# NeSC-IV/sage-icp

Measured on AMD Instinct MI355X. Metric: ICP frames/sec (120k-pt scan vs 1M-pt map), higher is better.
Workload: dtype f64

## Files before the change

sage-icp_amd/csrc/icp_body.h:

```cpp
#pragma once

namespace sageicp {

#ifndef SAGE_LOOP_FLAT_MINW
#define SAGE_LOOP_FLAT_MINW 8
#endif
#ifndef SAGE_SCAN_AHEAD
#define SAGE_SCAN_AHEAD 1
#endif
#ifndef SAGE_ROW_SHIFT_LAYER
#define SAGE_ROW_SHIFT_LAYER 1
#endif
#ifndef SAGE_ROW_SHIFT_MAXW
#define SAGE_ROW_SHIFT_MAXW 4
#endif

struct PairCompact {
    uint4 a, b;
    unsigned ka, oa;
    bool ha, hb;
};
struct PairFull {
    Point4 a, b;
    unsigned ka;
// ... 12 lines not shown

__device__ __forceinline__ unsigned icp_wave_of_stripe(const IcpParams &P, int wv, unsigned &stripe_id) {
    constexpr unsigned kStripe = SAGE_ICP_STRIPE;
    const unsigned xcd = blockIdx.x & 7u, jb = blockIdx.x >> 3;
    unsigned stripe = (jb / kStripe) * 8u + xcd;
    if (P.stripe_order) {
        const unsigned nstripes = gridDim.x / kStripe;
        switch (stripe * 4u / nstripes) {
            case 0: __builtin_amdgcn_s_setprio(3); break;
            case 1: __builtin_amdgcn_s_setprio(2); break;
            case 2: __builtin_amdgcn_s_setprio(1); break;
            default: break;
        }
        stripe = P.stripe_order[stripe];
    }
    stripe_id = stripe;
    const unsigned wg = stripe * kStripe + (jb % kStripe);
    return wg * static_cast<unsigned>(kIcpWavesPerBlock) + static_cast<unsigned>(wv);
}

template <bool GIVEN>
__device__ __forceinline__ void axis_gaps(double v, int k, double vs, double sc, double fs, double (&g)[3]) {
    const double below_hi = static_cast<double>(k <= 0 ? k - 1 : k) * vs;
    const double above_lo = static_cast<double>(k >= 0 ? k + 1 : k) * vs;
    const double slack = (GIVEN ? fs : 1e-9 * vs) + 1e-13 * fabs(v);
    const double lo = fmax((v - below_hi) - slack, 0.0);
    const double hi = fmax((above_lo - v) - slack, 0.0);
    g[0] = (lo * lo) * sc;
    g[1] = 0.0;
    g[2] = (hi * hi) * sc;
}

__device__ __forceinline__ float round_up_f32(double x) {
    return __uint_as_float(__float_as_uint(static_cast<float>(x)) + 1u);
}

template <int LW>
__device__ __forceinline__ bool reduce_argmin(double best, unsigned bkey, bool valid, const uint32_t *lrow, unsigned &mkey, unsigned &woff) {
    constexpr int W = 1 << LW, SH = 5;
    const double m = seg_min_f64<W>(best);
    const unsigned mine = (best == m) ? bkey : 0xFFFFFFFFu;
    mkey = seg_min_u32<W>(mine);
    const bool found = valid && mkey != 0xFFFFFFFFu;
    woff = (lrow[found ? mkey >> 8 : 0u] >> 8) * (kUnitPoints * 32u) + ((mkey & 255u) << SH);
    return found;
}

struct LoopStaged {
    unsigned qslot;
    double fx, fy, fz, fl;
    unsigned prev_key, prev_off;
    unsigned kx, ky, kz, occ;
    int pli;
};

template <int LW, bool FUSED, bool FILT, bool PERSIST = false, bool FLATQ = false, int HALF = 0>
__device__ __forceinline__ void icp_body(const IcpParams &P, uint32_t *smem, LoopGroup *G = nullptr, const double *pose = nullptr,
                                         LoopStaged *S = nullptr) {
    static_assert(!PERSIST || FUSED, "the persistent loop always accumulates");
    static_assert(PERSIST ? (HALF == 1 || HALF == 2) : HALF == 0, "k_loop runs the pass in two halves, k_icp in one");
    constexpr int W = 1 << LW;
    constexpr int QW = 64 >> LW;
    constexpr int SH = 5;
    PROBE_NN_BEGIN(np);
    PROBE_DELAY_BEGIN(t0);
    int lane;
    if constexpr (PERSIST) {
        unsigned l;
        asm volatile("v_mbcnt_lo_u32_b32 %0, -1, 0\n\tv_mbcnt_hi_u32_b32 %0, -1, %0" : "=v"(l));
        lane = static_cast<int>(l);
    } else {
        lane = static_cast<int>(threadIdx.x & 63u);
    }
    const int wv = __builtin_amdgcn_readfirstlane(static_cast<int>(threadIdx.x >> 6));
    if (FUSED && !PERSIST) {
        if (threadIdx.x == 0) {
            smem[kWgArrive] = 0u;
            smem[kWgGo] = 0u;
        }
        if (threadIdx.x < 2u * kWgAccWords) smem[kWgAcc + threadIdx.x] = 0u;
        if (threadIdx.x < 12u && !(P.chain && P.chain_iter > 0))
            reinterpret_cast<double *>(smem + kWgPose)[threadIdx.x] = threadIdx.x < 9u ? P.st->R[threadIdx.x] : P.st->T[4u + threadIdx.x - 9u];
        __syncthreads();
    }
    uint32_t *wl;
    if constexpr (PERSIST) wl = G->rows;
    else wl = smem + kWgHeaderWords + static_cast<unsigned>(wv) * icp_wave_words(LW);

    unsigned wave_id, stripe_id = 0u;
    if constexpr (PERSIST) wave_id = G->slot;
    else wave_id = icp_wave_of_stripe(P, wv, stripe_id);

    const int qw = lane >> LW;
    const unsigned ci = static_cast<unsigned>(lane) & (W - 1u);
    unsigned q, qslot = 0u, bslot = 0u;
    if constexpr (PERSIST) {
        if constexpr (HALF == 1) {
            bslot = G->perm[G->unit * (QW / 4) + static_cast<unsigned>(qw >> 2)];
            qslot = bslot * 4u + (static_cast<unsigned>(qw) & 3u);
        } else {
            qslot = S->qslot;
        }
        q = G->q_first + qslot;
    } else {
        q = wave_id * QW + static_cast<unsigned>(qw);
    }
    const bool valid = q < static_cast<unsigned>(P.n);
    const unsigned qc = valid ? q : 0u;
    uint32_t *lrow = wl + (PERSIST ? qslot : static_cast<unsigned>(qw)) * kRowLdsStride;
    const uint32_t *grow = P.rows + static_cast<size_t>(qc) * kRowWords;

    const __amdgpu_buffer_rsrc_t pts = __builtin_amdgcn_make_buffer_rsrc(
        const_cast<Point4 *>(P.pts), 0, static_cast<int>(P.pts_bytes), 0x00020000);

    const __amdgpu_buffer_rsrc_t cands = __builtin_amdgcn_make_buffer_rsrc(
        const_cast<uint4 *>(P.cand), 0, static_cast<int>(P.cand_bytes), 0x00020000);
    constexpr int SHC = FILT ? 4 : 5;

    constexpr int NP = (7 + W - 1) / W;
    uint4 rk;
    uint2 prev = make_uint2(0xFFFFFFFFu, 0u);
    Point4 f;
    uint4 pc0 = make_uint4(0u, 0u, 0u, 0u), pc1 = pc0, pc2 = pc0, pc3 = pc0, pc4 = pc0, pc5 = pc0, pc6 = pc0;
    uint32_t *lst = nullptr;
    if constexpr (PERSIST) {
        lst = G->state + qslot * kLoopStateWords;
        if constexpr (HALF == 1) {
            const uint4 fa = *reinterpret_cast<const uint4 *>(lst), fb = *reinterpret_cast<const uint4 *>(lst + 4);
            const uint4 pk = *reinterpret_cast<const uint4 *>(lst + kStPrev);
            const uint2 ko = *reinterpret_cast<const uint2 *>(lst + kStPrev + 4);
            S->qslot = qslot;
            S->fx = __hiloint2double(static_cast<int>(fa.y), static_cast<int>(fa.x));
            S->fy = __hiloint2double(static_cast<int>(fa.w), static_cast<int>(fa.z));
            S->fz = __hiloint2double(static_cast<int>(fb.y), static_cast<int>(fb.x));
            S->fl = __hiloint2double(static_cast<int>(fb.w), static_cast<int>(fb.z));
            S->prev_key = pk.x; S->prev_off = pk.y;
            S->kx = pk.z; S->ky = pk.w; S->kz = ko.x; S->occ = ko.y;
            S->pli = static_cast<int>(S->fl);
            return;
        }
        f.x = S->fx; f.y = S->fy; f.z = S->fz; f.l = S->fl;
        prev = make_uint2(S->prev_key, S->prev_off);
        rk = make_uint4(S->kx, S->ky, S->kz, S->occ);
    } else {
        rk = *reinterpret_cast<const uint4 *>(grow + kRowKey);
        if (FUSED) prev = P.nn_prev[qc];
        f = P.frame[qc];
        auto row_piece = [&](int k) {
            const unsigned p = min(ci + static_cast<unsigned>(W * k), 6u);
            return *reinterpret_cast<const uint4 *>(grow + 4u * p);
        };
        pc0 = row_piece(0); pc1 = pc0; pc2 = pc0; pc3 = pc0; pc4 = pc0; pc5 = pc0; pc6 = pc0;
        if (NP > 1) pc1 = row_piece(1);
        if (NP > 2) pc2 = row_piece(2);
        if (NP > 3) pc3 = row_piece(3);
        if (NP > 4) pc4 = row_piece(4);
        if (NP > 5) pc5 = row_piece(5);
        if (NP > 6) pc6 = row_piece(6);
    }
    PROBE_DELAY_WAIT(P, t0);
    if constexpr (FUSED && !PERSIST) {
        if (P.chain && P.chain_iter > 0) {
            if (wv == 0) chain_wait_pose(P, smem, lane);
            __syncthreads();
            if (smem[kWgGo]) return;
        }
    }
    PROBE_LOOP_POSE_USE(PERSIST, G);
    const Query s = [&]() {
        if constexpr (PERSIST) {
            return make_query<(W >= 4)>(f, pose, pose + 9, 1, P.voxel_size, P.inv_voxel_size, static_cast<unsigned>(lane));
        } else if constexpr (FUSED) {
            const double *lpose = reinterpret_cast<const double *>(smem + kWgPose);
            return make_query<(W >= 4)>(f, lpose, lpose + 9, P.apply_pose, P.voxel_size, P.inv_voxel_size, threadIdx.x);
        } else {
            return make_query<(W >= 4)>(f, P.st->R, P.st->T + 4, P.apply_pose, P.voxel_size, P.inv_voxel_size, threadIdx.x);
        }
    }();
    const bool stale = valid && (static_cast<uint32_t>(s.kx) != rk.x || static_cast<uint32_t>(s.ky) != rk.y ||
                                 static_cast<uint32_t>(s.kz) != rk.z);
    unsigned occ = rk.w;
    NN_T(np, 0);
    LP_T(PERSIST, G, 0);
    if constexpr (!PERSIST) {
        auto stage = [&](int k, const uint4 &v) {
            const unsigned p = ci + static_cast<unsigned>(W * k);
            if (p < 7u) *reinterpret_cast<uint4 *>(lrow + 4u * p) = v;
        };
        stage(0, pc0);
        if (NP > 1) stage(1, pc1);
        if (NP > 2) stage(2, pc2);
        if (NP > 3) stage(3, pc3);
        if (NP > 4) stage(4, pc4);
// ... 103 lines not shown
                        for (int j = j0; j < j0 + NB && j < NV; ++j) {
                            const int v = static_cast<int>(ci) + W * j;
                            if (reuse[j]) tally(v, ow[j]);
                            else finish(v, sl[j], e[j]);
                        }
                    }
                }
                if (nearv && prev.x != 0xFFFFFFFFu) {
                    const int vo = static_cast<int>(prev.x >> 8);
                    const int a = vo / 9 - dx, b = (vo / 3) % 3 - dy, c = vo % 3 - dz;
                    const bool in = static_cast<unsigned>(a) <= 2u && static_cast<unsigned>(b) <= 2u &&
                                    static_cast<unsigned>(c) <= 2u;
                    prev.x = in ? (static_cast<unsigned>(a * 9 + b * 3 + c) << 8) | (prev.x & 255u) : 0xFFFFFFFFu;
                } else {
                    prev.x = 0xFFFFFFFFu;
                }
            } else {
                prev.x = 0xFFFFFFFFu;
#pragma unroll 1
                for (int k0 = 0; k0 < NV; k0 += 3) {
                    const int v0 = static_cast<int>(ci) + W * k0;
                    const int v1 = k0 + 1 < NV ? v0 + W : 27, v2 = k0 + 2 < NV ? v0 + 2 * W : 27;
                    uint32_t s0, s1, s2;
                    int4 e0, e1, e2;
                    start(v0, s0, e0);
                    start(v1, s1, e1);
                    start(v2, s2, e2);
                    finish(v0, s0, e0);
                    finish(v1, s1, e1);
                    finish(v2, s2, e2);
                }
            }
            o = seg_or_u32<W>(o);
            cq = seg_add_u32<W>(cq);
            occ = o;
            if (ci == 0u) {
                lrow[kRowCq] = cq;
                if constexpr (!PERSIST) {
                    uint4 t;
                    t.x = static_cast<uint32_t>(s.kx); t.y = static_cast<uint32_t>(s.ky);
                    t.z = static_cast<uint32_t>(s.kz); t.w = o;
                    *reinterpret_cast<uint4 *>(P.rows + static_cast<size_t>(q) * kRowWords + kRowKey) = t;
                    P.rows[static_cast<size_t>(q) * kRowWords + kRowCq] = cq;
                }
            }
            if constexpr (PERSIST) {
                if (ci == 0u) {
                    *reinterpret_cast<uint2 *>(lst + kStKey) = make_uint2(static_cast<uint32_t>(s.kx), static_cast<uint32_t>(s.ky));
                    *reinterpret_cast<uint2 *>(lst + kStKey + 2) = make_uint2(static_cast<uint32_t>(s.kz), o);
                    lst[kStPrev] = prev.x;
                }
            }
        }
    }
    if constexpr (PERSIST) {
        __builtin_amdgcn_fence(__ATOMIC_ACQ_REL, "wavefront");
        prev.x = lst[opaque_v(kStPrev)];
    }
    if (!valid) occ = 0u;

    double gx[3], gy[3], gz[3];
    {
        const double vs = P.voxel_size, sc = P.prune_scale;
        double fs = 0.0;
        if constexpr (PERSIST) fs = reinterpret_cast<const LoopArgs *>(&P)->face_slack;
        axis_gaps<PERSIST>(s.x, s.kx, vs, sc, fs, gx);
        axis_gaps<PERSIST>(s.y, s.ky, vs, sc, fs, gy);
        axis_gaps<PERSIST>(s.z, s.kz, vs, sc, fs, gz);
    }
    NN_T(np, 1);
    LP_T(PERSIST, G, 1);

    double best = P.dist_init;
    unsigned bkey = 0xFFFFFFFFu;
    const int pli = HALF == 2 ? S->pli : static_cast<int>(s.l);
    const double th = P.sem_th;
    unsigned npairs = 0u;

    unsigned k = ci, kend = 0u, off = 0u;
    unsigned pk = 0u, needs = 0u, wn = 0u;
    auto evaluate = [&](const Point4 &nb, bool on, unsigned key) {
        const double dx = nb.x - s.x, dy = nb.y - s.y, dz = nb.z - s.z;
        double d = SAGE_SQNORM3_NN(dx * dx, dy * dy, dz * dz);
        const bool same = static_cast<int>(nb.l) == pli || fabs(nb.l * s.l) < 1.0;
        const double ds = d * th;
        d = same ? ds : d;
        d = __hiloint2double(on ? __double2hiint(d) : 0x7FF80000, __double2loint(d));
        const bool lt = d < best, eq = d == best, kl = key < bkey;
        const bool take = lt | (eq & kl);
        best = min_f64(best, d);
        bkey = take ? key : bkey;
    };

    const float qx = static_cast<float>(s.x), qy = static_cast<float>(s.y), qz = static_cast<float>(s.z);
    const float plab = static_cast<float>(pli);
    const bool q_zero = pli == 0;
    bool unknown = false;
    double slack = 0.0;
    if constexpr (FILT) {
        const bool q_exact = s.l == trunc(s.l) && fabs(s.l) < 16777216.0;
        unknown = !q_exact || (P.cand_flags[0] & 1u);
        const double ex = fabs(s.x) + 4.0 * P.voxel_size, ey = fabs(s.y) + 4.0 * P.voxel_size,
                     ez = fabs(s.z) + 4.0 * P.voxel_size;
        slack = (ex * ex + (ey * ey + ez * ez)) * P.filt_slack;
    }
    double fb = best;
    float Ts = 0.0f, Td = 0.0f, Tmax = 0.0f;
    auto set_thresholds = [&]() {
        if constexpr (!FILT) return;
        float a = round_up_f32(fb * P.filt_inv_same + slack), b = round_up_f32(fb * P.filt_inv_diff + slack);
        float m = a > b ? a : b;
        if (a != a || b != b) m = __uint_as_float(0x7FC00000u);
        if (unknown) a = b = m;
        Ts = a; Td = b; Tmax = m;
    };
    typedef float f2 __attribute__((ext_vector_type(2)));
    auto dist32 = [&](const uint4 &c, float &dl) {
        const f2 u = f2{__uint_as_float(c.x), __uint_as_float(c.y)} - f2{qx, qy};
        const f2 v = f2{__uint_as_float(c.z), __uint_as_float(c.w)} - f2{qz, plab};
        const f2 sq = u * u;
        dl = v.y;
        return __builtin_fmaf(v.x, v.x, sq.x) + sq.y;
    };
    auto tight = [&](const uint4 &c, float d, float dl) {
        const bool same = (dl == 0.0f) | (__uint_as_float(c.w) == 0.0f) | q_zero;
        return !(d > (same ? Ts : Td));
    };

    constexpr bool FLAT = PERSIST ? (W >= SAGE_LOOP_FLAT_MINW) : FLATQ;
    constexpr bool AHEAD = SAGE_SCAN_AHEAD != 0 && !FLAT && (PERSIST ? W >= 4 : (FUSED || FILT));
    constexpr unsigned kNeedEnd = 0x80000000u;
    using Pair = std::conditional_t<FLAT, std::conditional_t<FILT, PairCompactFlat, PairFullFlat>,
                                    std::conditional_t<FILT, PairCompact, PairFull>>;
    auto scan = [&](unsigned need, const Point4 *seed, bool seeded, unsigned seed_key) {
        auto next = [&](bool &h, unsigned &key, unsigned &o) {
            while (k >= kend && need) {
                const unsigned e = k - kend;
                const unsigned v = static_cast<unsigned>(__builtin_ctz(need));
                need &= need - 1u;
                const uint32_t w = lrow[v];
                kend = (v << 8) | (w & 255u);
                k = (v << 8) + e;
                off = (((w >> 8) * kUnitPoints) + e) << SHC;
                npairs += w & 255u;
            }
            h = k < kend;
            key = k;
            o = off;
            k += h ? static_cast<unsigned>(W) : 0u;
            off += h ? static_cast<unsigned>(W) << SHC : 0u;
        };
        auto pair_hb = [&](unsigned p) { return static_cast<int>(p) < -static_cast<int>(static_cast<unsigned>(W) << 16); };
        auto issue = [&](Pair &n, bool &more) {
            if constexpr (FLAT) {
                unsigned oa, ob;
                next(n.ha, n.ka, oa);
                next(n.hb, n.kb, ob);
// ... 53 lines not shown
            if constexpr (FILT) n.oa = off;
            const unsigned oa = n.ha ? off : 0u;
            if constexpr (FILT) {
                n.a = load_cand(cands, oa);
                n.b = load_cand(cands, oa, W << SHC);
            } else {
                const unsigned ob = n.hb ? off + (static_cast<unsigned>(W) << SHC) : 0u;
                n.a = load_point(pts, oa);
                n.b = load_point(pts, ob);
            }
            __builtin_amdgcn_sched_barrier(0);
            k += 2u * W;
            off += (2u * W) << SHC;
            more = (k < kend) | (need != 0u);
            }
        };
        auto consume = [&](const Pair &n) {
            unsigned kb;
            const unsigned ka = AHEAD ? n.ka & 0xFFFFu : n.ka;
            const bool ha = AHEAD ? static_cast<int>(n.ka) < 0 : n.ha, hb = AHEAD ? pair_hb(n.ka) : n.hb;
            if constexpr (FLAT) kb = n.kb; else kb = ka + W;
            if constexpr (!FILT) {
                evaluate(n.a, ha, ka);
                evaluate(n.b, hb, kb);
            } else {
            float dla, dlb;
            const float da = dist32(n.a, dla), db = dist32(n.b, dlb);
            const bool la = ha & !(da > Tmax) & (ka != bkey), lb = hb & !(db > Tmax) & (kb != bkey);
            PROBE_NN_CONSUME(np);
            if (__ballot(la | lb)) {
            const bool pa = la & tight(n.a, da, dla), pb = lb & tight(n.b, db, dlb);
            if (__ballot(pa | pb)) {
                PROBE_NN_EXACT(np, pa, pb);
                unsigned ob;
                if constexpr (FLAT) ob = n.ob; else ob = n.oa + (static_cast<unsigned>(W) << SHC);
                const Point4 ea = load_point(pts, pa ? n.oa << 1 : 0u);
                const Point4 eb = load_point(pts, pb ? ob << 1 : 0u);
                evaluate(ea, pa, ka);
                evaluate(eb, pb, kb);
                fb = min_f64(fb, best);
                set_thresholds();
            }
            }
            }
        };
        Pair A, B;
        bool more = false;
        if constexpr (AHEAD) {
            pk = 0u;
            off = 0u;
            needs = need | kNeedEnd;
            wn = lrow[__builtin_ctz(needs)];
        }
        issue(A, more);
        if (seed) evaluate(*seed, seeded, seed_key);
        fb = min_f64(fb, best);
        set_thresholds();
        for (;;) {
            issue(B, more);
            consume(A);
            issue(A, more);
            consume(B);
            if (!__ballot((AHEAD ? static_cast<int>(A.ka) < 0 : A.ha) | more)) break;
        }
    };

    constexpr unsigned kHome = 13u;
    bool merged = false;
    if constexpr (PERSIST) {
        const bool seeded = valid && prev.x != 0xFFFFFFFFu;
        const Point4 pp = *reinterpret_cast<const Point4 *>(lst + 8);
        evaluate(pp, seeded, prev.x);
        merged = seeded;
        const unsigned first = seeded ? 0u : (occ & (1u << kHome));
        if (__ballot(first != 0u)) scan(first, nullptr, false, 0u);
    } else if (FUSED) {
        const bool seeded = valid && prev.x != 0xFFFFFFFFu;
        const Point4 pp = load_point(pts, seeded ? prev.y : 0u);
        scan(occ & (1u << kHome), &pp, seeded, prev.x);
    } else {
        scan(occ & (1u << kHome), nullptr, false, 0u);
    }
    NN_T(np, 2);
    LP_T(PERSIST, G, 2);
    const double bound = seg_min_f64<W>(best);
    fb = bound;
    unsigned need = P.keep_all;
    if constexpr (W >= 4) {
        const unsigned a = (PERSIST ? static_cast<unsigned>(lane_now()) : ci) & 3u;
        const double ga = a == 0u ? gx[0] : (a == 2u ? gx[2] : 0.0);
        unsigned layer = 0u;
#pragma unroll
        for (int b = 0; b < 3; ++b) {
#pragma unroll
            for (int c = 0; c < 3; ++c) {
                const double lb = ga + (gy[b] + gz[c]);
                layer |= (lb <= bound) ? (1u << (3 * b + c)) : 0u;
            }
        }
        layer = (a < 3u && ci < 4u) ? layer << (9u * a) : 0u;
        layer |= dpp_u32<kDppXor1>(layer);
        layer |= dpp_u32<kDppXor2>(layer);
        if (W >= 8) layer |= dpp_u32<kDppHalfMirror>(layer);
        if (W >= 16) layer |= dpp_u32<kDppMirror>(layer);
        need |= layer & ~(1u << kHome);
    } else {
#pragma unroll
        for (int v = 0; v < 27; ++v) {
            if (v == static_cast<int>(kHome)) continue;
            const double lb = gx[v / 9] + (gy[(v / 3) % 3] + gz[v % 3]);
            need |= (lb <= bound) ? (1u << v) : 0u;
        }
    }
    LP_T(PERSIST, G, 3);
    scan((merged ? (need | (1u << kHome)) : (need & ~(1u << kHome))) & occ, nullptr, false, 0u);
    LP_T(PERSIST, G, 4);
    if constexpr (PERSIST) {
        lane = lane_now();
        const unsigned qe = static_cast<unsigned>(lane) >> LW;
        const unsigned bs = G->perm[G->unit * (QW / 4) + (qe >> 2)];
        lst = G->state + (bs * 4u + (qe & 3u)) * kLoopStateWords;
        if (valid && ci == 0u)
            (void)__hip_atomic_fetch_max(G->work + bs, npairs + (stale ? 48u : 0u), __ATOMIC_RELAXED, __HIP_MEMORY_SCOPE_WORKGROUP);
    }

    unsigned mkey, woff;
    const bool found = reduce_argmin<LW>(best, bkey, valid, lrow, mkey, woff);
    NN_T(np, 3);
    LP_T(PERSIST, G, 5);

    if (P.counters) {
        const unsigned long long ab = (valid && ci == 0u)
                                          ? (static_cast<unsigned long long>(lrow[kRowCq]) << 32) | npairs : 0ull;
        unsigned lo = static_cast<unsigned>(ab), hi = static_cast<unsigned>(ab >> 32);
        lo += dpp_u32<kDppXor1>(lo);        hi += dpp_u32<kDppXor1>(hi);
        lo += dpp_u32<kDppXor2>(lo);        hi += dpp_u32<kDppXor2>(hi);
        lo += dpp_u32<kDppHalfMirror>(lo);  hi += dpp_u32<kDppHalfMirror>(hi);
        lo += dpp_u32<kDppMirror>(lo);      hi += dpp_u32<kDppMirror>(hi);
        unsigned b = 0u, a = 0u;
#pragma unroll
        for (int r = 0; r < 4; ++r) {
            b += static_cast<unsigned>(__builtin_amdgcn_readlane(static_cast<int>(lo), 16 * r));
            a += static_cast<unsigned>(__builtin_amdgcn_readlane(static_cast<int>(hi), 16 * r));
        }
        if (lane == 0 && wave_id < P.nwaves) {
            (void)__hip_atomic_fetch_add(&P.counters[2u * wave_id], static_cast<unsigned long long>(a),
                                         __ATOMIC_RELAXED, __HIP_MEMORY_SCOPE_AGENT);
            (void)__hip_atomic_fetch_add(&P.counters[2u * wave_id + 1u], static_cast<unsigned long long>(b),
                                         __ATOMIC_RELAXED, __HIP_MEMORY_SCOPE_AGENT);
        }
    }

    if (!FUSED) {
        if (valid && ci == 0u) P.nn_idx[q] = found ? static_cast<int>(woff >> SH) : -1;
    } else {
        if constexpr (!PERSIST) {
            if (valid && ci == 0u) P.nn_prev[q] = make_uint2(found ? mkey : 0xFFFFFFFFu, woff);
        }
        Point4 g;
        if constexpr (PERSIST) {
            const bool changed = found && mkey != lst[opaque_v(kStPrev)];
            g = *reinterpret_cast<const Point4 *>(lst + 8);
            if (__ballot(changed)) {
                const Point4 t = load_point(pts, changed ? woff : 0u);
                if (changed) {
                    g = t;
                    if (ci == 0u) *reinterpret_cast<Point4 *>(lst + 8) = t;
                }
            }
            if (ci == 0u) *reinterpret_cast<uint2 *>(lst + kStPrev) = make_uint2(found ? mkey : 0xFFFFFFFFu, woff);
            LP_T(PERSIST, G, 6);
        }
        PROBE_NN_WORK(P, q, valid && ci == 0u, npairs);
        constexpr int K = kCount >> LW;
        double t[K];
        if constexpr (!PERSIST) g = load_point(pts, found ? woff : 0u);
        const double rx0 = s.x - g.x, ry0 = s.y - g.y, rz0 = s.z - g.z;
        const bool use = found && SAGE_SQNORM3_ACCEPT(rx0 * rx0, ry0 * ry0, rz0 * rz0) <= P.accept_r2;
        {
            const double r2 = SAGE_SQNORM3_RESID(rx0 * rx0, ry0 * ry0, rz0 * rz0);
            const double k = P.kernel;
            const double den = k + r2;
            const double wq = (k * k) / (den * den);
            const bool z = W == 1;
            const double w = !z || use ? wq : 0.0;
            const double sx = !z || use ? s.x : 0.0, sy = !z || use ? s.y : 0.0, sz = !z || use ? s.z : 0.0;
            const double rx = !z || use ? rx0 : 0.0, ry = !z || use ? ry0 : 0.0, rz = !z || use ? rz0 : 0.0;
            const double wsx = w * sx, wsy = w * sy, wsz = w * sz;
            double u[kCount];
            u[kW] = w;
            u[kWsx] = wsx; u[kWsy] = wsy; u[kWsz] = wsz;
            u[kWxx] = wsx * sx; u[kWxy] = wsx * sy; u[kWxz] = wsx * sz;
            u[kWyy] = wsy * sy; u[kWyz] = wsy * sz; u[kWzz] = wsz * sz;
            u[kWrx] = w * rx; u[kWry] = w * ry; u[kWrz] = w * rz;
            u[kWcx] = w * (sy * rz - sz * ry);
            u[kWcy] = w * (sz * rx - sx * rz);
            u[kWcz] = w * (sx * ry - sy * rx);
#pragma unroll
            for (int kk = 0; kk < K; ++kk) {
                double v = u[kk];
#pragma unroll
                for (int l = 1; l < W; ++l) v = ci == static_cast<unsigned>(l) ? u[l * K + kk] : v;
                t[kk] = z || use ? v : 0.0;
            }
        }
        const unsigned pairs = static_cast<unsigned>(__popcll(__ballot(use && ci == 0u)));
        if constexpr (PERSIST) {
            wave_terms_to_wgacc<LW, true>(t, pairs, lane, G->red, G->wgacc, kDigitLimitCounted, P.acc_scale);
            PROBE_LOOP_WAVE_STATS(smem, valid, ci, npairs, stale, lane);
            LP_T(PERSIST, G, 7);
            return;
        }
        if (P.stripe_work) {
            unsigned mx = valid ? npairs : 0u;
#pragma unroll
            for (int d = 1; d < 64; d <<= 1) mx = max(mx, static_cast<unsigned>(__shfl_xor(mx, d, 64)));
            if (lane == 0) (void)__hip_atomic_fetch_max(&P.stripe_work[stripe_id], mx, __ATOMIC_RELAXED, __HIP_MEMORY_SCOPE_AGENT);
        }
        {
            unsigned long long *wgacc = reinterpret_cast<unsigned long long *>(smem + kWgAcc);
            wave_terms_to_wgacc<LW>(t, pairs, lane, reinterpret_cast<double *>(wl), wgacc, P.digit_limit, P.acc_scale);
            unsigned prior = 0u;
            __atomic_signal_fence(__ATOMIC_SEQ_CST);
            if (lane == 0)
                prior = __hip_atomic_fetch_add(&smem[kWgArrive], 1u, __ATOMIC_RELAXED, __HIP_MEMORY_SCOPE_WORKGROUP);
            __atomic_signal_fence(__ATOMIC_SEQ_CST);
            prior = __builtin_amdgcn_readfirstlane(prior);
            if (prior == kIcpWavesPerBlock - 1u) {
                if (P.chain)
                    wgacc_flush<true>(wgacc, &P.chain->acc32[P.chain_iter & 1][blockIdx.x & (kChainReplicas - 1)][0], nullptr);
// ... 11 lines not shown
```

sage-icp_amd/csrc/kernels.h:

```cpp
#pragma once

#include <hip/hip_runtime.h>

#include "sageicp_types.h"

namespace sageicp {

constexpr int kRowWords = 32;
constexpr int kRowCq = 27, kRowKey = 28, kRowOcc = 31;
constexpr int kRowLdsStride = 36;

struct LoopShared;
struct IcpParams {
    const Point4 *frame;
    int n;
    const IcpState *st;
    int check_done;
    int apply_pose;
    double voxel_size;
    double inv_voxel_size;
    uint32_t *rows;
    const Slot *table;
    uint32_t mask;
    const Point4 *pts;
// ... 38 lines not shown
#endif
constexpr int kIcpWavesPerBlock = SAGE_ICP_WAVES;
int icp_blocks_for(int n, int lw);
size_t icp_lds_bytes(int lw);
void launch_rows(const IcpParams &p, hipStream_t s);
void launch_derive_cand(const Slot *table, uint32_t nslots, const Point4 *pts, uint4 *cand, uint64_t nslots_pts,
                        uint32_t *flags, hipStream_t s);
void launch_icp(const IcpParams &p, int lw, bool fused, hipStream_t s);

struct GnParams {
    const Point4 *src;
    const Point4 *tgt;
    int n;
    double kernel;
    double *partials;
};
int launch_gn(const GnParams &p, hipStream_t s);

constexpr int kAccReplicas = 32;
constexpr int kAccWords = 64;
constexpr int kAccValues = 17;
struct FinParams {
    IcpState *st;
    const double *partials;
    long long *acc;
    double acc_unscale;
    int nparts;
    int mode;
    int standalone;
    P2pParams p2p;
};
void launch_fin(const FinParams &p, hipStream_t s);

#ifndef SAGE_LOOP_REPLICAS
#define SAGE_LOOP_REPLICAS 8
#endif
constexpr int kLoopReplicas = SAGE_LOOP_REPLICAS;
constexpr int kLoopPoseGranules = 25;
constexpr int kLoopPoseCopies = 8;
constexpr int kLoopPoseStride = 32;
constexpr int kChainReplicas = 32;
struct LoopShared {
    long long acc[2][kLoopReplicas][kAccWords];
    unsigned long long pose[kLoopPoseCopies][kLoopPoseStride];
    unsigned long long abort_word[16];
    unsigned long long go[16];
    long long acc32[2][kChainReplicas][kAccWords];
};
struct LoopParams {
    LoopShared *sh;
    IcpState *st;
    int nw;
    int gpw;
    int wgs;
    int contiguous;
    uint32_t xcd_first[9];
    unsigned long long timeout_ticks;
    unsigned long long count_timeout_ticks;
    int max_iterations;
    unsigned long long epoch;
    double T0[7];
    double acc_unscale;
    int shared_loop;
    int prio;
    int deal;
    int copies;
    int pose_map;
    IcpProgress *progress;
};
struct LoopArgs {
    IcpParams P;
    LoopParams L;
    double face_slack;
};
#ifndef SAGE_LOOP_OCC
#define SAGE_LOOP_OCC 7
#endif
constexpr int kLoopMaxWavesHost = 8;
constexpr int kLoopStripeHost = 4;
constexpr int kLoopStateWords = 24;
size_t loop_lds_bytes(int lw, int nw, int gpw);
int loop_blocks_per_cu(int lw, bool filter, int nw, size_t lds);
void launch_loop(const IcpParams &p, const LoopParams &l, int lw, hipStream_t s);
void launch_loop_solve(const LoopParams &l, const P2pParams &x, hipStream_t s);

constexpr int kMaxPartials = 1 << 16;
constexpr uint64_t kMaxQueries = (1ull << 26) - 4;

void launch_tf(Point4 *pts, int n, const IcpState *st, hipStream_t s);
void launch_scatter_points(const uint32_t *idx, const Point4 *vals, uint32_t n, Point4 *pts,
                           hipStream_t s);
void launch_scatter_slots(const uint32_t *idx, const Slot *vals, uint32_t n, Slot *table,
                          hipStream_t s);
void launch_scatter_u32(const uint32_t *idx, const uint32_t *vals, uint32_t n, uint32_t *dst, hipStream_t s);
void launch_sum_counters(const unsigned long long *c, int n, IcpState *st, hipStream_t s);

struct VdsParams {
    const Point4 *in;
    int n;
    int do_crop;
    double max_range, min_range, label_max_range;
    int n_groups;
    const int *group_counts;
    const int *group_labels;
    double group_vs[8];
    double scale;
    unsigned long long *keys;
    uint32_t *winner;
    uint32_t mask;
    Point4 *tmp;
    uint32_t *slot_of;
    uint32_t *sort_key;
    uint32_t *sort_val;
    int *overflow;
    unsigned long long *out_keys;
};
size_t vds_sort_temp_bytes(int n);
void launch_vds_permute(const Point4 *in, const uint32_t *perm, uint32_t n, Point4 *out, hipStream_t s);
hipError_t voxel_downsample_device(const VdsParams &P, void *sort_temp, size_t sort_temp_bytes,
                                   uint32_t *d_n_kept, Point4 *out, hipStream_t s);

struct DeskewTangent {
    double v[6];
};
void launch_deskew(const Point4 *in, Point4 *out, const double *ts, int n, const DeskewTangent &d, hipStream_t s);

// ... 52 lines not shown
```

sage-icp_amd/csrc/kernels.hip:

```cpp

#include <hip/hip_runtime.h>

#include <algorithm>
#include <cfloat>
#include <cstdlib>
#include <type_traits>
#include <vector>

#ifndef SAGE_ICP_STRIPE
#define SAGE_ICP_STRIPE 8
#endif
#ifndef SAGE_ICP_OCC
#define SAGE_ICP_OCC 6
#endif

#include "kernels.h"
#include "se3_math.h"
#include "sageicp_types.h"
#include "probes.h"

namespace sageicp {


template <int CTRL>
// ... 594 lines not shown
            if (fused) hipLaunchKernelGGL((k_icp<LW, true, false, F>), g, b, lds, s, p);
            else hipLaunchKernelGGL((k_icp<LW, false, false, F>), g, b, lds, s, p);
        }
    };
    if constexpr (kBoth) {
        if (flat) go(std::true_type{});
        else go(std::false_type{});
    } else if constexpr (LW >= 3) {
        go(std::true_type{});
    } else {
        go(std::false_type{});
    }
}
void launch_icp(const IcpParams &p, int lw, bool fused, hipStream_t s) {
    if (p.n <= 0) return;
    switch (lw) {
        case 0: launch_icp_lw<0>(p, fused, s); break;
        case 1: launch_icp_lw<1>(p, fused, s); break;
        case 2: launch_icp_lw<2>(p, fused, s); break;
        case 3: launch_icp_lw<3>(p, fused, s); break;
        default: launch_icp_lw<4>(p, fused, s); break;
    }
}

size_t loop_lds_bytes(int lw, int nw, int gpw) {
    return sizeof(uint32_t) * LoopLds<size_t>(lw, static_cast<size_t>(nw), static_cast<size_t>(gpw)).end;
}
static const void *loop_kernel(int lw, bool filter) {
#define SAGE_LOOP_K(LW_, F_) reinterpret_cast<const void *>(&k_loop<LW_, F_>)
    switch (lw) {
        case 1: return filter ? SAGE_LOOP_K(1, true) : SAGE_LOOP_K(1, false);
        case 2: return filter ? SAGE_LOOP_K(2, true) : SAGE_LOOP_K(2, false);
        case 3: return filter ? SAGE_LOOP_K(3, true) : SAGE_LOOP_K(3, false);
        case 4: return filter ? SAGE_LOOP_K(4, true) : SAGE_LOOP_K(4, false);
        default: return nullptr;
    }
#undef SAGE_LOOP_K
}
int loop_blocks_per_cu(int lw, bool filter, int nw, size_t lds) {
    if (nw < 1 || nw > kLoopMaxWaves || lds > 160 * 1024) return 0;
    const void *k = loop_kernel(lw, filter);
    if (!k) return 0;
    if (lds > 64 * 1024 && hipFuncSetAttribute(k, hipFuncAttributeMaxDynamicSharedMemorySize, 160 * 1024) != hipSuccess) return 0;
    int nb = 0;
    if (hipOccupancyMaxActiveBlocksPerMultiprocessor(&nb, k, 64 * nw, lds) != hipSuccess) return 0;
    return nb;
}
void launch_loop(const IcpParams &p, const LoopParams &l, int lw, hipStream_t s) {
    const size_t lds = loop_lds_bytes(lw, l.nw, l.gpw);
    LoopArgs a;
    a.P = p;
    a.L = l;
    a.face_slack = 1e-9 * p.voxel_size;
    void *args[] = {&a};
#ifdef SAGE_LOOP_INGRID
    (void)hipLaunchKernel(loop_kernel(lw, p.filter != 0), dim3(l.wgs + 1), dim3(64 * l.nw), args, lds, s);
#else
    (void)hipLaunchKernel(loop_kernel(lw, p.filter != 0), dim3(l.wgs), dim3(64 * l.nw), args, lds, s);
#endif
}
void launch_loop_solve(const LoopParams &l, const P2pParams &x, hipStream_t s) {
    SolveArgs a;
    a.L = l;
    a.X = x;
    if (l.copies == kChainReplicas) hipLaunchKernelGGL(k_loop_solve<kChainReplicas>, dim3(1), dim3(64), 0, s, a);
    else hipLaunchKernelGGL(k_loop_solve<kLoopReplicas>, dim3(1), dim3(64), 0, s, a);
}

int launch_gn(const GnParams &p, hipStream_t s) {
    long blocks = (static_cast<long>(p.n) + 255) / 256;
    if (blocks > 128) blocks = 128;
    if (blocks < 1) blocks = 1;
    hipLaunchKernelGGL(k_gn, dim3(static_cast<int>(blocks)), dim3(256), 0, s, p);
    return static_cast<int>(blocks);
}

void launch_fin(const FinParams &p, hipStream_t s) {
    hipLaunchKernelGGL(k_fin, dim3(1), dim3(kFinThreads), 0, s, p);
}

void launch_tf(Point4 *pts, int n, const IcpState *st, hipStream_t s) {
    if (n <= 0) return;
    hipLaunchKernelGGL(k_tf, dim3((n + 255) / 256), dim3(256), 0, s, pts, n, st);
}

}
```

sage-icp_amd/csrc/loop_kernel.h:

```cpp
#pragma once

namespace sageicp {


__device__ __forceinline__ int exchange_sums_wave(double *S, const P2pParams &X, unsigned long long g) {
    const int lane = static_cast<int>(threadIdx.x & 63u);
    const int slot = static_cast<int>(g & 1ull);
    const unsigned long long tag = g + 1ull;
    if (lane < kNumSums) {
        const double v = S[lane];
        for (int r = 0; r < X.nranks; ++r)
            __hip_atomic_store(&X.block[r]->sums[slot][X.rank][lane], v, __ATOMIC_RELAXED, __HIP_MEMORY_SCOPE_SYSTEM);
    }
    asm volatile("s_waitcnt vmcnt(0)" ::: "memory");
    __builtin_amdgcn_fence(__ATOMIC_RELEASE, "");
    asm volatile("s_waitcnt vmcnt(0)" ::: "memory");
    if (lane == 0)
        for (int r = 0; r < X.nranks; ++r)
            __hip_atomic_store(&X.block[r]->flag[X.rank], tag, __ATOMIC_RELAXED, __HIP_MEMORY_SCOPE_SYSTEM);
    P2pBlock *mine = X.block[X.rank];
    bool late = false, gone = false;
    if (lane < X.nranks) {
        const unsigned long long t0 = __builtin_amdgcn_s_memrealtime();
        while (__hip_atomic_load(&mine->flag[lane], __ATOMIC_RELAXED, __HIP_MEMORY_SCOPE_SYSTEM) < tag) {
// ... 325 lines not shown
        smem[kLpFirst + static_cast<unsigned>(wv)] = (((hw >> 4) & 3u) + (hw & 15u)) % static_cast<unsigned>(nw);
    }
    for (unsigned i = threadIdx.x; i < 2u * kWgAccWords; i += blockDim.x) smem[kLpAcc + i] = 0u;
    for (unsigned i = threadIdx.x; i < nblk_max; i += blockDim.x) {
        perm0[i] = i;
        work0[i] = 0u;
    }
    for (unsigned sl = threadIdx.x; sl < gcnt * QW; sl += blockDim.x) {
        const unsigned q = g0 * QW + sl;
        const Point4 f = P.frame[q < static_cast<unsigned>(P.n) ? q : 0u];
        {
            uint32_t *lst = state0 + sl * kLoopStateWords;
            *reinterpret_cast<Point4 *>(lst) = f;
            Point4 z;
            z.x = z.y = z.z = z.l = 0.0;
            *reinterpret_cast<Point4 *>(lst + 8) = z;
            *reinterpret_cast<uint4 *>(lst + kStPrev) = make_uint4(0xFFFFFFFFu, 0u, static_cast<uint32_t>(kNoVoxel),
                                                                   static_cast<uint32_t>(kNoVoxel));
            *reinterpret_cast<uint4 *>(lst + kStPrev + 4) = make_uint4(static_cast<uint32_t>(kNoVoxel), 0u, 0u, 0u);
        }
    }
    __syncthreads();
    if (L.deal) {
        unsigned claimed = 0u, kept = 0u, table[kLoopMaxWaves];
        for (int w2 = 0; w2 < nw; ++w2) {
            const unsigned pr = smem[kLpFirst + static_cast<unsigned>(w2)];
            table[w2] = pr;
            if (!((claimed >> pr) & 1u)) { claimed |= 1u << pr; kept |= 1u << w2; }
        }
        for (int w2 = 0; w2 < nw; ++w2)
            if (!((kept >> w2) & 1u)) {
                const unsigned pr = static_cast<unsigned>(__builtin_ctz(~claimed));
                table[w2] = pr;
                claimed |= 1u << pr;
            }
        __syncthreads();
        if (threadIdx.x == 0) {
            for (int w2 = 0; w2 < nw; ++w2) smem[kLpFirst + static_cast<unsigned>(w2)] = table[w2];
            smem[kLpNext] = static_cast<unsigned>(nw);
        }
        __syncthreads();
    }
    static_assert(kLoopMaxWaves <= 8, "k_loop keeps the wave's index in three bits");
    const unsigned who = (blockIdx.x << 3) | static_cast<unsigned>(wv);
    PROBE_LOOP_BEGIN(lp);


    for (;;) {
        PROBE_LOOP_IT(it, smem);
        constexpr unsigned kNoUnit = 0xFFFFFFFFu;
        LoopStaged S{};
        PROBE_LOOP_UNIT_VAR(t_unit);
        auto group_of = [&](unsigned u, const LoopArgs &B) {
            const LoopLds<unsigned> lds(LW, static_cast<unsigned>(B.L.nw), static_cast<unsigned>(B.L.gpw));
            const unsigned first_unit = opaque_s(g0);
            LoopGroup G;
            G.rows = smem + lds.rows;
            G.state = smem + lds.state;
            G.perm = smem + lds.perm;
            G.work = smem + lds.work;
            G.unit = u;
            G.red = reinterpret_cast<double *>(smem + lds.red + (opaque_s(who) & 7u) * loop_red_words());
            G.wgacc = reinterpret_cast<unsigned long long *>(smem + kLpAcc);
            G.q_first = first_unit * QW;
            G.slot = first_unit + u;
            return G;
        };
        auto stage = [&](unsigned u) {
            auto kb = __builtin_amdgcn_kernarg_segment_ptr();
            asm volatile("" : "+s"(kb));
            const LoopArgs &B = *(const LoopArgs *)(kb);
            if (B.L.prio) loop_set_priority(u, B.L.nw, B.L.prio);
            PROBE_LOOP_UNIT_BEGIN(it, u, B.L.nw, t_unit);
            LoopGroup G = group_of(u, B);
            icp_body<LW, true, FILT, true, false, 1>(B.P, smem, &G, nullptr, &S);
        };
        auto ka = __builtin_amdgcn_kernarg_segment_ptr();
        asm volatile("" : "+s"(ka));
        unsigned gi = kNoUnit;
        if (((const LoopArgs *)(ka))->L.deal) {
            gi = static_cast<unsigned>(__builtin_amdgcn_readfirstlane(static_cast<int>(smem[kLpFirst + (opaque_s(who) & 7u)])));
            if (gi >= opaque_s(gcnt)) gi = kNoUnit;
        }
        if (gi != kNoUnit) stage(gi);
        {
            const LoopParams &L = ((const LoopArgs *)(ka))->L;
            const unsigned itn = (opaque_s(who) & 7u) == 0u ? static_cast<unsigned>(__builtin_amdgcn_readfirstlane(static_cast<int>(smem[kLpIter]))) : 0u;
            if (itn != 0u) {
                LoopShared *sh = L.sh;
                const int lane = lane_now();
                const unsigned wg = opaque_s(who) >> 3;
                const unsigned long long tag = static_cast<unsigned long long>(itn);
                const unsigned long long t0 = __builtin_amdgcn_s_memrealtime();
                unsigned long long g = tag << 32;
                bool aborted = false;
                for (;;) {
                    if (lane < kLoopPoseGranules) g = ld_agent(&sh->pose[loop_pose_copy(L.pose_map, wg)][lane]);
                    const bool ok = (g >> 32) == tag;
                    if (__all(ok)) break;
                    unsigned long long ab = 0ull;
                    if (lane == 0) ab = ld_agent(&sh->abort_word[0]);
                    const bool late = __builtin_amdgcn_s_memrealtime() - t0 > L.timeout_ticks;
                    if (__any(ab != 0ull) || late) {
                        if (lane == 0 && late) {
                            st_agent(&sh->abort_word[0], 1ull);
                            L.st->loop_aborted = 1;
                        }
                        aborted = true;
                        break;
                    }
                    __builtin_amdgcn_s_sleep(SAGE_LOOP_POLL_SLEEP);
                    if (L.wgs > 1024) __builtin_amdgcn_s_sleep(SAGE_LOOP_POLL_SLEEP);
                }
                if (aborted) {
                    if (lane == 0) smem[kLpDone] = 2u;
                } else {
                    if (lane < 24) smem[kLpPose + static_cast<unsigned>(lane)] = static_cast<uint32_t>(g);
                    if (lane == 24) smem[kLpDone] = static_cast<uint32_t>(g);
                }
                LOOP_STAMP_WG(itn - 1u, 1);
            }
        }
        PROBE_LOOP_WAIT_BEGIN(t_b);
        __syncthreads();
        PROBE_LOOP_WAITED(lp, t_b);
        if (smem[kLpDone]) break;
        for (;;) {
            if (gi != kNoUnit) {
                auto kb = __builtin_amdgcn_kernarg_segment_ptr();
                asm volatile("" : "+s"(kb));
                const LoopArgs &B = *(const LoopArgs *)(kb);
                LoopGroup G = group_of(opaque_s(gi), B);
                PROBE_LOOP_PASS_BEGIN(lp, G);
                icp_body<LW, true, FILT, true, false, 2>(B.P, smem, &G, reinterpret_cast<const double *>(smem + kLpPose), &S);
                PROBE_LOOP_UNIT_END(lp, G, it, gi, B.L.nw, static_cast<int>(opaque_s(who) & 7u), lane_now(), t_unit);
            }
            gi = 0u;
            if (lane_now() == 0)
                gi = __hip_atomic_fetch_add(&smem[kLpNext], 1u, __ATOMIC_RELAXED, __HIP_MEMORY_SCOPE_WORKGROUP);
            gi = static_cast<unsigned>(__builtin_amdgcn_readfirstlane(static_cast<int>(gi)));
            if (gi >= opaque_s(gcnt)) break;
            stage(gi);
        }
        PROBE_LOOP_MARK(t_a);
        auto kc = __builtin_amdgcn_kernarg_segment_ptr();
        asm volatile("" : "+s"(kc));
        const LoopParams &L = ((const LoopArgs *)(kc))->L;
        LoopShared *sh = L.sh;
        const int lane = lane_now();
        const unsigned me = opaque_s(who), wg = me >> 3;
        unsigned prior = 0u;
        __atomic_signal_fence(__ATOMIC_SEQ_CST);
        if (lane == 0)
            prior = __hip_atomic_fetch_add(&smem[kLpArrive], 1u, __ATOMIC_RELAXED, __HIP_MEMORY_SCOPE_WORKGROUP);
        __atomic_signal_fence(__ATOMIC_SEQ_CST);
        prior = static_cast<unsigned>(__builtin_amdgcn_readfirstlane(static_cast<int>(prior)));
        const bool last = prior == static_cast<unsigned>(L.nw) - 1u;
        if (last) {
            const int it = __builtin_amdgcn_readfirstlane(static_cast<int>(smem[kLpIter]));
            wgacc_flush<true, true>(reinterpret_cast<unsigned long long *>(smem + kLpAcc), &sh->acc[it & 1][wg & (kLoopReplicas - 1)][0],
                                    &sh->acc[it & 1][0][kAccWords - 1]);
            if (lane == 0) {
                smem[kLpArrive] = 0u;
                smem[kLpIter] = static_cast<unsigned>(it) + 1u;
                smem[kLpNext] = L.deal ? static_cast<unsigned>(L.nw) : 0u;
            }
            const unsigned nblk = opaque_s(gcnt) * BPW;
            if (nblk <= 64u && nblk > BPW) {
                const LoopLds<unsigned> lds(LW, static_cast<unsigned>(L.nw), static_cast<unsigned>(L.gpw));
                uint32_t *perm = smem + lds.perm, *work = smem + lds.work;
                __builtin_amdgcn_fence(__ATOMIC_ACQ_REL, "wavefront");
                const unsigned i = static_cast<unsigned>(lane);
                const unsigned wi = i < nblk ? work[i] : 0u;
                unsigned rank = 0u;
                for (unsigned j = 0; j < nblk; ++j) {
                    const unsigned wj = work[j];
                    rank += (wj > wi || (wj == wi && j < i)) ? 1u : 0u;
                }
                __builtin_amdgcn_fence(__ATOMIC_ACQ_REL, "wavefront");
                if (i < nblk) {
                    perm[rank] = i;
                    work[i] = 0u;
                }
            }
            PROBE_LOOP_WG_INFO(smem, it, lane);
            LOOP_STAMP_WG(it, 0);
        }
        PROBE_LOOP_CLOSED(lp, last, t_a);
        PROBE_LOOP_WAIT_BEGIN(t_c);
        __syncthreads();
        PROBE_LOOP_WAITED(lp, t_c);
    }
    PROBE_LOOP_END(lp);
}

}
```

Measured before the change: 247.6.

## Hoist kernel-argument and LDS seed loads earlier in persistent ICP loop

Precomputes LDS region offsets on the host and passes them as kernel arguments instead of recomputing the layout on device. In the persistent loop it issues scalar parameter loads and the previous-match seed point load earlier so their latency overlaps other work. It also caches the query's unknown-label flag in the staged state and reuses the previously read key. Adds a latency microbenchmark for scalar and LDS loads, and reorders LoopParams fields. Risks are higher register pressure and compiler scheduling changes.

```diff
diff --git a/profiles/micro/lgkm_latency.hip b/profiles/micro/lgkm_latency.hip
--- /dev/null
+++ b/profiles/micro/lgkm_latency.hip
@@ -0,0 +1,68 @@
+#include <hip/hip_runtime.h>
+#include <cstdio>
+#include <vector>
+
+struct Chase {
+    unsigned next[64];
+};
+
+__global__ void k_lat(Chase c, int rounds, unsigned long long *out) {
+    __shared__ __attribute__((aligned(16))) unsigned lds[256];
+    typedef __attribute__((address_space(3))) unsigned *lds_ptr;
+    const unsigned base = static_cast<unsigned>(reinterpret_cast<uintptr_t>((lds_ptr)lds));
+    for (unsigned i = threadIdx.x; i < 256u; i += blockDim.x) lds[i] = base + ((i * 4u + 4u) & 252u) * 4u;
+    __syncthreads();
+    auto ka = __builtin_amdgcn_kernarg_segment_ptr();
+    const unsigned long long r0 = __builtin_amdgcn_s_memrealtime();
+    unsigned long long t0 = __builtin_amdgcn_s_memtime(), acc = 0;
+    for (int k = 0; k < rounds; ++k) {
+        const unsigned long long a = __builtin_amdgcn_s_memtime();
+        acc += __builtin_amdgcn_s_memtime() - a;
+    }
+    const unsigned long long stamps = acc;
+    unsigned off = 0u;
+    t0 = __builtin_amdgcn_s_memtime();
+    for (int k = 0; k < rounds; ++k) asm volatile("s_load_dword %0, %1, %0\n\ts_waitcnt lgkmcnt(0)" : "+s"(off) : "s"(ka) : "memory");
+    const unsigned long long t_s = __builtin_amdgcn_s_memtime() - t0;
+    unsigned a = base + (threadIdx.x & 63u) * 16u;
+    t0 = __builtin_amdgcn_s_memtime();
+    for (int k = 0; k < rounds; ++k) asm volatile("ds_read_b32 %0, %0\n\ts_waitcnt lgkmcnt(0)" : "+v"(a) : : "memory");
+    const unsigned long long t_l = __builtin_amdgcn_s_memtime() - t0;
+    uint4 v = make_uint4(0u, 0u, 0u, 0u);
+    t0 = __builtin_amdgcn_s_memtime();
+    for (int k = 0; k < rounds; ++k) {
+        asm volatile("ds_read_b128 %0, %1\n\ts_waitcnt lgkmcnt(0)" : "=v"(v) : "v"(a) : "memory");
+        a = v.x;
+    }
+    const unsigned long long t_q = __builtin_amdgcn_s_memtime() - t0;
+    if (threadIdx.x == 0 && blockIdx.x == 0) {
+        out[0] = stamps;
+        out[1] = t_s;
+        out[2] = t_l;
+        out[3] = t_q;
+        out[4] = __builtin_amdgcn_s_memrealtime() - r0;
+        out[5] = off + a + v.y;
+    }
+}
+
+int main() {
+    Chase c;
+    for (unsigned i = 0; i < 64u; ++i) c.next[i] = ((i * 17u + 1u) & 63u) * 4u;
+    unsigned long long *out = nullptr;
+    if (hipMalloc(&out, 8 * sizeof(unsigned long long)) != hipSuccess) return 1;
+    const int rounds = 4096;
+    const int shapes[][2] = {{1, 64}, {256, 256}, {1792, 256}};
+    for (const auto &s : shapes) {
+        for (int rep = 0; rep < 2; ++rep) {
+            hipLaunchKernelGGL(k_lat, dim3(s[0]), dim3(s[1]), 0, 0, c, rounds, out);
+            if (hipDeviceSynchronize() != hipSuccess) return 1;
+        }
+        std::vector<unsigned long long> h(8);
+        if (hipMemcpy(h.data(), out, 8 * sizeof(unsigned long long), hipMemcpyDeviceToHost) != hipSuccess) return 1;
+        std::printf("%5d workgroups x %3d threads: s_memtime pair %6.1f | s_load (kernel arguments, hit) %6.1f | ds_read_b32 %6.1f | ds_read_b128 %6.1f "
+                    "cycles per dependent access (%llu ticks of 10 ns in all)\n",
+                    s[0], s[1], double(h[0]) / rounds, double(h[1]) / rounds, double(h[2]) / rounds, double(h[3]) / rounds, h[4]);
+    }
+    (void)hipFree(out);
+    return 0;
+}
diff --git a/sage-icp_amd/csrc/icp_body.h b/sage-icp_amd/csrc/icp_body.h
--- a/sage-icp_amd/csrc/icp_body.h
+++ b/sage-icp_amd/csrc/icp_body.h
@@ -88,6 +88,7 @@
     unsigned prev_key, prev_off;
     unsigned kx, ky, kz, occ;
     int pli;
+    bool unknown;
 };
 
 template <int LW, bool FUSED, bool FILT, bool PERSIST = false, bool FLATQ = false, int HALF = 0>
@@ -159,6 +160,9 @@
     Point4 f;
     uint4 pc0 = make_uint4(0u, 0u, 0u, 0u), pc1 = pc0, pc2 = pc0, pc3 = pc0, pc4 = pc0, pc5 = pc0, pc6 = pc0;
     uint32_t *lst = nullptr;
+    struct { double vs, th, init, fslack; } E{};
+    Point4 pp_seed;
+    constexpr bool kSeedEarly = PERSIST && !(FILT && W >= 8);
     if constexpr (PERSIST) {
         lst = G->state + qslot * kLoopStateWords;
         if constexpr (HALF == 1) {
@@ -173,8 +177,11 @@
             S->prev_key = pk.x; S->prev_off = pk.y;
             S->kx = pk.z; S->ky = pk.w; S->kz = ko.x; S->occ = ko.y;
             S->pli = static_cast<int>(S->fl);
+            if constexpr (FILT) S->unknown = !(S->fl == trunc(S->fl) && fabs(S->fl) < 16777216.0) || (P.cand_flags[0] & 1u);
             return;
         }
+        if constexpr (kSeedEarly) E.vs = P.voxel_size, E.th = P.sem_th, E.init = P.dist_init, E.fslack = P.filt_slack;
+        if constexpr (kSeedEarly) pp_seed = *reinterpret_cast<const Point4 *>(lst + 8);
         f.x = S->fx; f.y = S->fy; f.z = S->fz; f.l = S->fl;
         prev = make_uint2(S->prev_key, S->prev_off);
         rk = make_uint4(S->kx, S->ky, S->kz, S->occ);
@@ -384,16 +391,24 @@
                 }
             }
         }
-    }
-    if constexpr (PERSIST) {
-        __builtin_amdgcn_fence(__ATOMIC_ACQ_REL, "wavefront");
-        prev.x = lst[opaque_v(kStPrev)];
+        if constexpr (PERSIST) {
+            __builtin_amdgcn_fence(__ATOMIC_ACQ_REL, "wavefront");
+            prev.x = lst[opaque_v(kStPrev)];
+            const IcpParams *Pr = &P;
+            asm volatile("" : "+s"(Pr));
+            if constexpr (kSeedEarly) E.vs = Pr->voxel_size, E.th = Pr->sem_th, E.init = Pr->dist_init, E.fslack = Pr->filt_slack;
+            if constexpr (kSeedEarly) pp_seed = *reinterpret_cast<const Point4 *>(lst + opaque_v(8u));
+        }
+    }
+    if constexpr (PERSIST && !kSeedEarly) {
+        E.vs = P.voxel_size; E.th = P.sem_th; E.init = P.dist_init; E.fslack = P.filt_slack;
+        pp_seed = *reinterpret_cast<const Point4 *>(lst + 8);
     }
     if (!valid) occ = 0u;
 
     double gx[3], gy[3], gz[3];
     {
-        const double vs = P.voxel_size, sc = P.prune_scale;
+        const double vs = PERSIST ? E.vs : P.voxel_size, sc = P.prune_scale;
         double fs = 0.0;
         if constexpr (PERSIST) fs = reinterpret_cast<const LoopArgs *>(&P)->face_slack;
         axis_gaps<PERSIST>(s.x, s.kx, vs, sc, fs, gx);
@@ -403,10 +418,10 @@
     NN_T(np, 1);
     LP_T(PERSIST, G, 1);
 
-    double best = P.dist_init;
+    double best = PERSIST ? E.init : P.dist_init;
     unsigned bkey = 0xFFFFFFFFu;
     const int pli = HALF == 2 ? S->pli : static_cast<int>(s.l);
-    const double th = P.sem_th;
+    const double th = PERSIST ? E.th : P.sem_th;
     unsigned npairs = 0u;
 
     unsigned k = ci, kend = 0u, off = 0u;
@@ -430,11 +445,15 @@
     bool unknown = false;
     double slack = 0.0;
     if constexpr (FILT) {
-        const bool q_exact = s.l == trunc(s.l) && fabs(s.l) < 16777216.0;
-        unknown = !q_exact || (P.cand_flags[0] & 1u);
-        const double ex = fabs(s.x) + 4.0 * P.voxel_size, ey = fabs(s.y) + 4.0 * P.voxel_size,
-                     ez = fabs(s.z) + 4.0 * P.voxel_size;
-        slack = (ex * ex + (ey * ey + ez * ez)) * P.filt_slack;
+        if constexpr (HALF == 2) {
+            unknown = S->unknown;
+        } else {
+            const bool q_exact = s.l == trunc(s.l) && fabs(s.l) < 16777216.0;
+            unknown = !q_exact || (P.cand_flags[0] & 1u);
+        }
+        const double v4 = 4.0 * (PERSIST ? E.vs : P.voxel_size);
+        const double ex = fabs(s.x) + v4, ey = fabs(s.y) + v4, ez = fabs(s.z) + v4;
+        slack = (ex * ex + (ey * ey + ez * ez)) * (PERSIST ? E.fslack : P.filt_slack);
     }
     double fb = best;
     float Ts = 0.0f, Td = 0.0f, Tmax = 0.0f;
@@ -594,6 +613,7 @@
             needs = need | kNeedEnd;
             wn = lrow[__builtin_ctz(needs)];
         }
+        if constexpr (PERSIST && FILT) asm volatile("" ::"s"(P.filt_inv_same), "s"(P.filt_inv_diff));
         issue(A, more);
         if (seed) evaluate(*seed, seeded, seed_key);
         fb = min_f64(fb, best);
@@ -611,8 +631,7 @@
     bool merged = false;
     if constexpr (PERSIST) {
         const bool seeded = valid && prev.x != 0xFFFFFFFFu;
-        const Point4 pp = *reinterpret_cast<const Point4 *>(lst + 8);
-        evaluate(pp, seeded, prev.x);
+        evaluate(pp_seed, seeded, prev.x);
         merged = seeded;
         const unsigned first = seeded ? 0u : (occ & (1u << kHome));
         if (__ballot(first != 0u)) scan(first, nullptr, false, 0u);
@@ -657,11 +676,13 @@
     LP_T(PERSIST, G, 3);
     scan((merged ? (need | (1u << kHome)) : (need & ~(1u << kHome))) & occ, nullptr, false, 0u);
     LP_T(PERSIST, G, 4);
+    unsigned kprev = 0u;
     if constexpr (PERSIST) {
         lane = lane_now();
         const unsigned qe = static_cast<unsigned>(lane) >> LW;
         const unsigned bs = G->perm[G->unit * (QW / 4) + (qe >> 2)];
         lst = G->state + (bs * 4u + (qe & 3u)) * kLoopStateWords;
+        kprev = lst[opaque_v(kStPrev)];
         if (valid && ci == 0u)
             (void)__hip_atomic_fetch_max(G->work + bs, npairs + (stale ? 48u : 0u), __ATOMIC_RELAXED, __HIP_MEMORY_SCOPE_WORKGROUP);
     }
@@ -671,6 +692,9 @@
     NN_T(np, 3);
     LP_T(PERSIST, G, 5);
 
+    if constexpr (PERSIST) {
+        asm volatile("" ::"s"(P.counters), "s"(P.kernel), "s"(P.accept_r2));
+    }
     if (P.counters) {
         const unsigned long long ab = (valid && ci == 0u)
                                           ? (static_cast<unsigned long long>(lrow[kRowCq]) << 32) | npairs : 0ull;
@@ -701,7 +725,7 @@
         }
         Point4 g;
         if constexpr (PERSIST) {
-            const bool changed = found && mkey != lst[opaque_v(kStPrev)];
+            const bool changed = found && mkey != kprev;
             g = *reinterpret_cast<const Point4 *>(lst + 8);
             if (__ballot(changed)) {
                 const Point4 t = load_point(pts, changed ? woff : 0u);
@@ -718,6 +742,7 @@
         double t[K];
         if constexpr (!PERSIST) g = load_point(pts, found ? woff : 0u);
         const double rx0 = s.x - g.x, ry0 = s.y - g.y, rz0 = s.z - g.z;
+        if constexpr (PERSIST) __builtin_amdgcn_sched_barrier(0);
         const bool use = found && SAGE_SQNORM3_ACCEPT(rx0 * rx0, ry0 * ry0, rz0 * rz0) <= P.accept_r2;
         {
             const double r2 = SAGE_SQNORM3_RESID(rx0 * rx0, ry0 * ry0, rz0 * rz0);
diff --git a/sage-icp_amd/csrc/kernels.h b/sage-icp_amd/csrc/kernels.h
--- a/sage-icp_amd/csrc/kernels.h
+++ b/sage-icp_amd/csrc/kernels.h
@@ -114,6 +114,8 @@
     IcpState *st;
     int nw;
     int gpw;
+    int prio;
+    int deal;
     int wgs;
     int contiguous;
     uint32_t xcd_first[9];
@@ -124,8 +126,6 @@
     double T0[7];
     double acc_unscale;
     int shared_loop;
-    int prio;
-    int deal;
     int copies;
     int pose_map;
     IcpProgress *progress;
@@ -134,6 +134,7 @@
     IcpParams P;
     LoopParams L;
     double face_slack;
+    unsigned lds_perm, lds_state, lds_rows, lds_work, lds_red;
 };
 #ifndef SAGE_LOOP_OCC
 #define SAGE_LOOP_OCC 7
diff --git a/sage-icp_amd/csrc/kernels.hip b/sage-icp_amd/csrc/kernels.hip
--- a/sage-icp_amd/csrc/kernels.hip
+++ b/sage-icp_amd/csrc/kernels.hip
@@ -670,6 +670,12 @@
     a.P = p;
     a.L = l;
     a.face_slack = 1e-9 * p.voxel_size;
+    const LoopLds<unsigned> at(lw, static_cast<unsigned>(l.nw), static_cast<unsigned>(l.gpw));
+    a.lds_perm = at.perm;
+    a.lds_state = at.state;
+    a.lds_rows = at.rows;
+    a.lds_work = at.work;
+    a.lds_red = at.red;
     void *args[] = {&a};
 #ifdef SAGE_LOOP_INGRID
     (void)hipLaunchKernel(loop_kernel(lw, p.filter != 0), dim3(l.wgs + 1), dim3(64 * l.nw), args, lds, s);
diff --git a/sage-icp_amd/csrc/loop_kernel.h b/sage-icp_amd/csrc/loop_kernel.h
--- a/sage-icp_amd/csrc/loop_kernel.h
+++ b/sage-icp_amd/csrc/loop_kernel.h
@@ -401,15 +401,14 @@
         LoopStaged S{};
         PROBE_LOOP_UNIT_VAR(t_unit);
         auto group_of = [&](unsigned u, const LoopArgs &B) {
-            const LoopLds<unsigned> lds(LW, static_cast<unsigned>(B.L.nw), static_cast<unsigned>(B.L.gpw));
             const unsigned first_unit = opaque_s(g0);
             LoopGroup G;
-            G.rows = smem + lds.rows;
-            G.state = smem + lds.state;
-            G.perm = smem + lds.perm;
-            G.work = smem + lds.work;
+            G.rows = smem + B.lds_rows;
+            G.state = smem + B.lds_state;
+            G.perm = smem + B.lds_perm;
+            G.work = smem + B.lds_work;
             G.unit = u;
-            G.red = reinterpret_cast<double *>(smem + lds.red + (opaque_s(who) & 7u) * loop_red_words());
+            G.red = reinterpret_cast<double *>(smem + B.lds_red + (opaque_s(who) & 7u) * loop_red_words());
             G.wgacc = reinterpret_cast<unsigned long long *>(smem + kLpAcc);
             G.q_first = first_unit * QW;
             G.slot = first_unit + u;
@@ -516,8 +515,7 @@
             }
             const unsigned nblk = opaque_s(gcnt) * BPW;
             if (nblk <= 64u && nblk > BPW) {
-                const LoopLds<unsigned> lds(LW, static_cast<unsigned>(L.nw), static_cast<unsigned>(L.gpw));
-                uint32_t *perm = smem + lds.perm, *work = smem + lds.work;
+                uint32_t *perm = smem + ((const LoopArgs *)(kc))->lds_perm, *work = smem + ((const LoopArgs *)(kc))->lds_work;
                 __builtin_amdgcn_fence(__ATOMIC_ACQ_REL, "wavefront");
                 const unsigned i = static_cast<unsigned>(lane);
                 const unsigned wi = i < nblk ? work[i] : 0u;
```

After: 248.2, median of 3. Within noise of the previous version (+0.2%).
